# jnbraun/bcnn

Hardware: AMD Instinct MI355X
Metric: images/sec fwd+bwd (higher is better)
Workload: dtype f32; 1 GPU; ResNet-18 224x224 (BASELINE configs[2]), N=128 per GPU, fwd+bwd+SGD through bcnn_net C API; CIFAR-example topology + ImageNet stem, fc-1000; batch_per_gpu=128, global_batch=128, parallelism=dp1, comm=none (one rank)

## Files before the change

bcnn_amd/csrc/batchnorm.hip:

```cpp
#include "chan_reduce.h"
#include "batchnorm.h"
#include "bn_math.h"

namespace bcnn_hip {

#ifdef NT_STORES
#define BN_ST4(p, v) do { typedef float f4_ __attribute__((ext_vector_type(4))); const f4_ t_ = {(v).x, (v).y, (v).z, (v).w}; \
                          __builtin_nontemporal_store(t_, reinterpret_cast<f4_*>(p)); } while (0)
#else
#define BN_ST4(p, v) (*reinterpret_cast<float4*>(p) = (v))
#endif


static float4* bn_consts_scratch(int channels) {
    if (BCNN_EXP_ENV("BCNN_HIP_BN_NO_CONSTS")) return nullptr;
    return scratch_f4(SCRATCH_BN_CONSTS, (size_t)channels * 3);
}
__device__ __forceinline__ void bn_fwd_consts_store(float4* consts, int c, float mean, float var, const float* scale,
                                                    const float* bias) {
    if (!consts) return;
    const BnDiv rs = bn_divisor(sqrtf(var + 0.000001f));
    consts[2 * c] = make_float4(mean, rs.d, rs.r, scale[c]);
    consts[2 * c + 1] = make_float4(bias[c], 0.f, 0.f, 0.f);
}
__device__ __forceinline__ void bn_bwd_consts_store(float4* consts, int c, const float* mean, float var, float sc,
                                                    const float* fwd_bias, float dmean, float dvar, float fM) {
    if (!consts) return;
    const BnDiv rs5 = bn_divisor(sqrtf(var + 0.00001f)), rs6 = bn_divisor(sqrtf(var + 0.000001f));
    consts[3 * c] = make_float4(mean[c], sc, rs5.d, rs5.r);
    consts[3 * c + 1] = make_float4(rs6.d, rs6.r, fwd_bias ? fwd_bias[c] : 0.f, __fdiv_rn(dmean, fM));
    consts[3 * c + 2] = make_float4(dvar, 0.f, 0.f, 0.f);
}

struct StatsF {
    static constexpr int kInFlight = 4;
    const float* x;
    __device__ void operator()(long long off, int, float (&acc)[2]) const {
        const float v = x[off];
        acc[0] += v;
        acc[1] += v * v;
    }
    __device__ void vec4(long long off, int, float (&acc)[2]) const {
        const float4 v = *reinterpret_cast<const float4*>(x + off);
        acc[0] += (v.x + v.y) + (v.z + v.w);
        acc[1] += (v.x * v.x + v.y * v.y) + (v.z * v.z + v.w * v.w);
    }
};

__global__ void bn_stats_finalize_kernel(const float* __restrict__ partials, int C, int splits, int M,
                                         float* __restrict__ saved_mean, float* __restrict__ saved_var,
                                         float* __restrict__ run_mean, float* __restrict__ run_var,
                                         float4* __restrict__ consts, const float* __restrict__ scale,
                                         const float* __restrict__ bias, const float* __restrict__ mean_shift) {
    const int c = blockIdx.x * blockDim.x + threadIdx.x;
    if (c >= C) return;
    double s = 0.0, ss = 0.0;
    for (int i = 0; i < splits; ++i) {
        s += (double)partials[((long long)c * splits + i) * 2 + 0];
        ss += (double)partials[((long long)c * splits + i) * 2 + 1];
    }
    const float inv = 1.0f / (float)M;
    const float mean = __fmul_rn((float)s, inv);
    const float var = __fsub_rn(__fmul_rn((float)ss, inv), __fmul_rn(mean, mean));
    saved_mean[c] = mean;
    saved_var[c] = var;
    const float vis = mean_shift ? __fadd_rn(mean, mean_shift[c]) : mean;
    run_mean[c] = __fadd_rn(__fmul_rn(vis, 0.1f), __fmul_rn(run_mean[c], 0.9f));
    run_var[c] = __fadd_rn(__fmul_rn(var, 0.1f), __fmul_rn(run_var[c], 0.9f));
    bn_fwd_consts_store(consts, c, mean, var, scale, bias);
}

constexpr int kFinalizeThreads = 1024;
__global__ __launch_bounds__(kFinalizeThreads) void bn_stats_finalize_wide_kernel(
    const float* __restrict__ partials, int C, int splits, int M, float* __restrict__ saved_mean,
    float* __restrict__ saved_var, float* __restrict__ run_mean, float* __restrict__ run_var,
    float4* __restrict__ consts, const float* __restrict__ scale, const float* __restrict__ bias,
    const float* __restrict__ mean_shift) {
    constexpr int NW = kFinalizeThreads / 64;
    __shared__ double red[NW][2];
    const int lane = threadIdx.x & 63, wid = threadIdx.x >> 6;
    const int c = blockIdx.x;
    const float2* p = reinterpret_cast<const float2*>(partials) + (long long)c * splits;
    double s = 0.0, ss = 0.0;
    int i = threadIdx.x;
    for (; i + 3 * kFinalizeThreads < splits; i += 4 * kFinalizeThreads) {
        const float2 v0 = p[i], v1 = p[i + kFinalizeThreads], v2 = p[i + 2 * kFinalizeThreads], v3 = p[i + 3 * kFinalizeThreads];
        s += ((double)v0.x + (double)v1.x) + ((double)v2.x + (double)v3.x);
        ss += ((double)v0.y + (double)v1.y) + ((double)v2.y + (double)v3.y);
    }
    for (; i < splits; i += kFinalizeThreads) {
        const float2 v = p[i];
        s += (double)v.x;
        ss += (double)v.y;
    }
#pragma unroll
    for (int o = 32; o > 0; o >>= 1) { s += __shfl_xor(s, o); ss += __shfl_xor(ss, o); }
    if (lane == 0) { red[wid][0] = s; red[wid][1] = ss; }
    __syncthreads();
    if (threadIdx.x != 0) return;
    s = 0.0;
    ss = 0.0;
    for (int w = 0; w < NW; ++w) { s += red[w][0]; ss += red[w][1]; }
    const float inv = 1.0f / (float)M;
    const float mean = __fmul_rn((float)s, inv);
    const float var = __fsub_rn(__fmul_rn((float)ss, inv), __fmul_rn(mean, mean));
    saved_mean[c] = mean;
    saved_var[c] = var;
    const float vis = mean_shift ? __fadd_rn(mean, mean_shift[c]) : mean;
    run_mean[c] = __fadd_rn(__fmul_rn(vis, 0.1f), __fmul_rn(run_mean[c], 0.9f));
    run_var[c] = __fadd_rn(__fmul_rn(var, 0.1f), __fmul_rn(run_var[c], 0.9f));
    bn_fwd_consts_store(consts, c, mean, var, scale, bias);
}

struct BnApplyArgs {
    const float* x;
    float* y;
    float* ws;
    float* xn;
    const float* mean;
    const float* var;
    const float* scale;
    const float* bias;
    int C, HW, predict, act;
    long long total;
    const float* res;
    unsigned res_count;
    int act2;
    const float4* consts;
};

struct BnApplyBody {
    BnApplyArgs a;
    bool al;
    __device__ void operator()(unsigned off, int c, int cnt) const {
        float mean, sc, b;
        BnDiv rs;
        if (a.consts) {
            const float4 k0 = a.consts[2 * c], k1 = a.consts[2 * c + 1];
            mean = k0.x; rs.d = k0.y; rs.r = k0.z; sc = k0.w; b = k1.x;
        } else {
            mean = a.predict ? 0.f : a.mean[c];
            rs = bn_divisor(a.predict ? 1.f : sqrtf(a.var[c] + 0.000001f));
            sc = a.scale[c]; b = a.bias[c];
        }
        const bool side_ws = a.ws && a.ws != a.x, side_xn = a.xn && !a.predict;
        if (cnt == 4 && al && (off & 3u) == 0) {
            const float4 xv = *reinterpret_cast<const float4*>(a.x + off);
            float4 yv, nv;
            yv.x = bn_one(xv.x, mean, rs, sc, b, a.predict, a.act, &nv.x);
            yv.y = bn_one(xv.y, mean, rs, sc, b, a.predict, a.act, &nv.y);
            yv.z = bn_one(xv.z, mean, rs, sc, b, a.predict, a.act, &nv.z);
            yv.w = bn_one(xv.w, mean, rs, sc, b, a.predict, a.act, &nv.w);
            if (side_ws) *reinterpret_cast<float4*>(a.ws + off) = xv;
            if (side_xn) *reinterpret_cast<float4*>(a.xn + off) = nv;
            if (a.res) {
                if (off + 4 <= a.res_count) {
                    const float4 r = *reinterpret_cast<const float4*>(a.res + off);
                    yv.x += r.x; yv.y += r.y; yv.z += r.z; yv.w += r.w;
                } else if (off < a.res_count) {
                    yv.x += a.res[off];
                    if (off + 1 < a.res_count) yv.y += a.res[off + 1];
                    if (off + 2 < a.res_count) yv.z += a.res[off + 2];
                }
                yv.x = act_fwd_cheap(yv.x, a.act2, 0.f); yv.y = act_fwd_cheap(yv.y, a.act2, 0.f);
                yv.z = act_fwd_cheap(yv.z, a.act2, 0.f); yv.w = act_fwd_cheap(yv.w, a.act2, 0.f);
            }
            BN_ST4(a.y + off, yv);
        } else {
            for (int k = 0; k < cnt; ++k) {
                const float xv = a.x[off + k];
                float nv = 0.f;
                float yv = bn_one(xv, mean, rs, sc, b, a.predict, a.act, &nv);
                if (a.res) yv = act_fwd_cheap(yv + (off + k < a.res_count ? a.res[off + k] : 0.f), a.act2, 0.f);
                if (side_ws) a.ws[off + k] = xv;
                if (side_xn) a.xn[off + k] = nv;
                a.y[off + k] = yv;
            }
        }
    }
};

__device__ __forceinline__ float bn_recompute_y(float x, float m, const BnDiv& rs, float sc, float b, int act, const float* res,
                                                unsigned res_count, unsigned long long off) {
    float dummy;
    if (!res) return bn_one(x, m, rs, sc, b, 0, act, &dummy);
    float v = bn_one(x, m, rs, sc, b, 0, BCNN_HIP_ACT_NONE, &dummy);
    if (off < res_count) v += res[off];
    return act_fwd_cheap(v, act, 0.f);
}

struct BwdSumsF {
    static constexpr int kInFlight = 2;
    const float* dy;
    const float* y;
    const float* x;
    const float* mean;
    const float* fwd_bias;
    const float* var;
    const float* scale;
    int act, C, HW;
    const float* res;
    unsigned res_count;
    __device__ float fwd_y(float xv, int c, long long off) const {
        return bn_recompute_y(xv, mean[c], bn_divisor(sqrtf(var[c] + 0.000001f)), scale[c], fwd_bias[c], act, res, res_count,
                              (unsigned long long)off);
    }
    __device__ void operator()(long long off, int c, float (&acc)[2]) const {
        float g = dy[off];
        const float xv = x[off];
        if (act != BCNN_HIP_ACT_NONE) g *= act_bwd_cheap(fwd_bias ? fwd_y(xv, c, off) : y[off], act, 0.f);
        acc[0] += g;
        acc[1] += g * (xv - mean[c]);
    }
    __device__ void vec4(long long off, int c, float (&acc)[2]) const {
        const float m = mean[c];
        float4 g = *reinterpret_cast<const float4*>(dy + off);
        const float4 xv = *reinterpret_cast<const float4*>(x + off);
        if (act != BCNN_HIP_ACT_NONE) {
            float4 yv;
            if (fwd_bias) {
                const BnDiv rs = bn_divisor(sqrtf(var[c] + 0.000001f));
                const float sc = scale[c], b = fwd_bias[c];
                const unsigned long long o = (unsigned long long)off;
                yv.x = bn_recompute_y(xv.x, m, rs, sc, b, act, res, res_count, o);
                yv.y = bn_recompute_y(xv.y, m, rs, sc, b, act, res, res_count, o + 1);
                yv.z = bn_recompute_y(xv.z, m, rs, sc, b, act, res, res_count, o + 2);
                yv.w = bn_recompute_y(xv.w, m, rs, sc, b, act, res, res_count, o + 3);
            } else {
                yv = *reinterpret_cast<const float4*>(y + off);
            }
            g.x *= act_bwd_cheap(yv.x, act, 0.f); g.y *= act_bwd_cheap(yv.y, act, 0.f);
            g.z *= act_bwd_cheap(yv.z, act, 0.f); g.w *= act_bwd_cheap(yv.w, act, 0.f);
        }
        acc[0] += (g.x + g.y) + (g.z + g.w);
        acc[1] += (g.x * (xv.x - m) + g.y * (xv.y - m)) + (g.z * (xv.z - m) + g.w * (xv.w - m));
    }
};

__global__ void bn_bwd_finalize_kernel(const float* __restrict__ partials, int C, int splits,
                                       const float* __restrict__ scale, const float* __restrict__ var,
                                       float* __restrict__ dbias, float* __restrict__ dscales,
                                       float* __restrict__ dmean, float* __restrict__ dvar,
                                       float4* __restrict__ consts, const float* __restrict__ mean,
                                       const float* __restrict__ fwd_bias, float fM) {
    const int c = blockIdx.x * blockDim.x + threadIdx.x;
    if (c >= C) return;
    double s1 = 0.0, s2 = 0.0;
    for (int i = 0; i < splits; ++i) {
        s1 += (double)partials[((long long)c * splits + i) * 2 + 0];
        s2 += (double)partials[((long long)c * splits + i) * 2 + 1];
    }
    const float v = var[c], sc = scale[c];
    dbias[c] += (float)s1;
    dscales[c] += (float)(s2 / (double)sqrtf(v + 0.000001f));
    float md = (float)(s1 * (double)sc);
    float vd = (float)(s2 * (double)sc);
    md *= (-1.0f / sqrtf(v + 0.00001f));
    vd *= -0.5f / (v * sqrtf(v) + 0.00001f);
    dmean[c] = md;
    dvar[c] = vd;
    bn_bwd_consts_store(consts, c, mean, v, sc, fwd_bias, md, vd, fM);
}

__global__ __launch_bounds__(1024) void bn_bwd_finalize_wide_kernel(const float* __restrict__ partials, int C, int splits,
                                                                   const float* __restrict__ scale,
                                                                   const float* __restrict__ var, float* __restrict__ dbias,
                                                                   float* __restrict__ dscales, float* __restrict__ dmean,
                                                                   float* __restrict__ dvar, float4* __restrict__ consts,
                                                                   const float* __restrict__ mean,
                                                                   const float* __restrict__ fwd_bias, float fM) {
    __shared__ double red[16][2];
    const int lane = threadIdx.x & 63, wid = threadIdx.x >> 6, c = blockIdx.x;
    const float2* p = reinterpret_cast<const float2*>(partials) + (long long)c * splits;
    double s1 = 0.0, s2 = 0.0;
    int i = threadIdx.x;
    for (; i + 3 * 1024 < splits; i += 4 * 1024) {
        const float2 v0 = p[i], v1 = p[i + 1024], v2 = p[i + 2048], v3 = p[i + 3072];
        s1 += ((double)v0.x + (double)v1.x) + ((double)v2.x + (double)v3.x);
        s2 += ((double)v0.y + (double)v1.y) + ((double)v2.y + (double)v3.y);
    }
    for (; i < splits; i += 1024) {
        const float2 v = p[i];
        s1 += (double)v.x;
        s2 += (double)v.y;
    }
#pragma unroll
    for (int o = 32; o > 0; o >>= 1) { s1 += __shfl_xor(s1, o); s2 += __shfl_xor(s2, o); }
    if (lane == 0) { red[wid][0] = s1; red[wid][1] = s2; }
    __syncthreads();
    if (threadIdx.x != 0) return;
    s1 = 0.0;
    s2 = 0.0;
    for (int w = 0; w < 16; ++w) { s1 += red[w][0]; s2 += red[w][1]; }
    const float v = var[c], sc = scale[c];
    dbias[c] += (float)s1;
    dscales[c] += (float)(s2 / (double)sqrtf(v + 0.000001f));
    float md = (float)(s1 * (double)sc);
    float vd = (float)(s2 * (double)sc);
    md *= (-1.0f / sqrtf(v + 0.00001f));
    vd *= -0.5f / (v * sqrtf(v) + 0.00001f);
    dmean[c] = md;
    dvar[c] = vd;
    bn_bwd_consts_store(consts, c, mean, v, sc, fwd_bias, md, vd, fM);
}

struct BnBwdApplyArgs {
    float* dy;
    float* dx;
    const float* y;
    const float* x;
    const float* mean;
    const float* var;
    const float* scale;
    const float* dmean;
    const float* dvar;
    const float* fwd_bias;
    int C, HW, act, M;
    long long total;
    int keep_dy;
    const float* res;
    unsigned res_count;
    const float4* consts;
    float rM;
};

struct BnBwdApplyBody {
    BnBwdApplyArgs a;
    bool al;
    __device__ void operator()(unsigned off, int c, int cnt) const {
        const BnDiv fM{(float)a.M, a.rM};
        const bool use_act = a.act != BCNN_HIP_ACT_NONE, use_y = use_act && a.fwd_bias == nullptr;
        float mean, sc, fb, dmm, dv;
        BnDiv rs, rs_fwd;
        if (a.consts) {
            const float4 k0 = a.consts[3 * c], k1 = a.consts[3 * c + 1], k2 = a.consts[3 * c + 2];
            mean = k0.x; sc = k0.y; rs.d = k0.z; rs.r = k0.w;
            rs_fwd.d = k1.x; rs_fwd.r = k1.y; fb = k1.z; dmm = k1.w; dv = k2.x;
        } else {
            mean = a.mean[c]; sc = a.scale[c];
            rs = bn_divisor(sqrtf(a.var[c] + 0.00001f));
            rs_fwd = bn_divisor(use_act && !use_y ? sqrtf(a.var[c] + 0.000001f) : 1.0f);
            fb = a.fwd_bias ? a.fwd_bias[c] : 0.f;
            dmm = __fdiv_rn(a.dmean[c], fM.d); dv = a.dvar[c];
        }
        if (cnt == 4 && al && (off & 3u) == 0) {
            const float4 g = *reinterpret_cast<const float4*>(a.dy + off);
            const float4 xv = *reinterpret_cast<const float4*>(a.x + off);
            float4 yv = make_float4(0.f, 0.f, 0.f, 0.f);
            if (use_y) yv = *reinterpret_cast<const float4*>(a.y + off);
            else if (use_act) {
                yv.x = bn_recompute_y(xv.x, mean, rs_fwd, sc, fb, a.act, a.res, a.res_count, off);
                yv.y = bn_recompute_y(xv.y, mean, rs_fwd, sc, fb, a.act, a.res, a.res_count, off + 1ull);
                yv.z = bn_recompute_y(xv.z, mean, rs_fwd, sc, fb, a.act, a.res, a.res_count, off + 2ull);
                yv.w = bn_recompute_y(xv.w, mean, rs_fwd, sc, fb, a.act, a.res, a.res_count, off + 3ull);
            }
            float4 o;
            o.x = bn_bwd_one(g.x, yv.x, xv.x, mean, rs, sc, dmm, dv, fM, a.act);
            o.y = bn_bwd_one(g.y, yv.y, xv.y, mean, rs, sc, dmm, dv, fM, a.act);
            o.z = bn_bwd_one(g.z, yv.z, xv.z, mean, rs, sc, dmm, dv, fM, a.act);
            o.w = bn_bwd_one(g.w, yv.w, xv.w, mean, rs, sc, dmm, dv, fM, a.act);
            if (!a.keep_dy) BN_ST4(a.dy + off, o);
            if (a.dx) BN_ST4(a.dx + off, o);
        } else {
            for (int k = 0; k < cnt; ++k) {
                const float xk = a.x[off + k];
                const float yk = use_y ? a.y[off + k]
                                       : (use_act ? bn_recompute_y(xk, mean, rs_fwd, sc, fb, a.act, a.res, a.res_count, off + k) : 0.f);
                const float o = bn_bwd_one(a.dy[off + k], yk, xk, mean, rs, sc, dmm, dv, fM, a.act);
                if (!a.keep_dy) a.dy[off + k] = o;
                if (a.dx) a.dx[off + k] = o;
            }
        }
    }
};

void batchnorm_forward_impl(const BnFwdCall& f) {
    const int n = f.e.n, c = f.e.c, hw = f.e.hw, mode = f.mode;
    const long long M = (long long)n * hw, total = M * c;
    if (!total) return;
    const bool have_pre = f.pre && f.pre->splits > 0 && mode == BCNN_HIP_MODE_TRAIN;
    KTimer kt(K_BN_FWD, 0.0, 4.0 * ((have_pre ? 0.0 : 1.0) + (f.stats_only ? 0.0 : 2.0)) * (double)total);
    const int act = act_is_cheap(f.act) ? f.act : BCNN_HIP_ACT_NONE;
    BnApplyArgs a;
    a.x = f.x; a.y = f.y; a.ws = f.workspace; a.xn = f.x_norm; a.scale = f.p.scales; a.bias = f.p.bias;
    a.C = c; a.HW = hw; a.act = act; a.total = total;
    a.res = nullptr; a.res_count = 0; a.act2 = BCNN_HIP_ACT_NONE;
    if (f.res) {
        a.res = f.res->res;
        a.res_count = (unsigned)(f.res->count < (size_t)total ? f.res->count : (size_t)total);
        a.act2 = f.res->act;
    }
    a.predict = (mode == BCNN_HIP_MODE_PREDICT);
    a.mean = f.run.run_mean; a.var = f.run.run_var;
    a.consts = nullptr;
    float4* consts = (mode == BCNN_HIP_MODE_TRAIN && !f.stats_only) ? bn_consts_scratch(c) : nullptr;
    if (mode == BCNN_HIP_MODE_PREDICT) a.ws = nullptr;
    if (mode == BCNN_HIP_MODE_VALID) a.xn = nullptr;
    if (mode == BCNN_HIP_MODE_TRAIN) {
        if (have_pre) {
            bn_stats_finalize_wide_kernel<<<c, kFinalizeThreads, 0, current_stream()>>>(
                f.pre->partials, c, f.pre->splits, (int)M, f.saved_mean, f.saved_var, f.run.run_mean, f.run.run_var, consts,
                f.p.scales, f.p.bias, f.mean_shift);
        } else {
            const int splits = chan_splits(c, M);
            float* part = scratch(SCRATCH_REDUCE, (size_t)c * splits * 2);
            launch_chan_reduce<2>(StatsF{f.x}, c, hw, M, splits, part);
            bn_stats_finalize_kernel<<<ceil_div(c, 256), 256, 0, current_stream()>>>(
                part, c, splits, (int)M, f.saved_mean, f.saved_var, f.run.run_mean, f.run.run_var, consts, f.p.scales, f.p.bias,
                f.mean_shift);
        }
        KERNEL_CHECK();
        a.mean = f.saved_mean; a.var = f.saved_var; a.consts = consts;
    }
    if (f.stats_only) return;
#ifdef BCNN_HIP_EXPERIMENT
    static const int skip_fw = getenv("BCNN_HIP_SKIP_SWEEPS") ? atoi(getenv("BCNN_HIP_SKIP_SWEEPS")) : 0;
    if (!(skip_fw & 4))
#endif
    launch_chan_map(BnApplyBody{a, al16(f.x) && al16(f.y) && al16(a.ws) && al16(a.xn) && al16(a.res)}, n, c, hw);
    if (f.act != act) bcnn_hip_activation_forward(f.y, (size_t)total, f.act, nullptr, hw, c);
}

}

using namespace bcnn_hip;

extern "C" {

void bcnn_hip_batchnorm_forward_stats(const float* x, float* y, float* run_mean, float* run_var, const float* scales,
                                      const float* bias, float* saved_mean, float* saved_var, float* x_norm,
                                      float* workspace, int n, int c, int hw, int mode, int act, const float* stats,
                                      int splits) {
    ConvStats st;
    st.partials = const_cast<float*>(stats); st.splits = stats ? splits : 0; st.capacity = 0;
    BnFwdCall f{};
    f.x = x; f.y = y; f.workspace = workspace; f.x_norm = x_norm; f.mode = mode; f.act = act; f.pre = &st;
    f.e.n = n; f.e.c = c; f.e.hw = hw; f.p.scales = scales; f.p.bias = bias;
    f.saved_mean = saved_mean; f.saved_var = saved_var; f.run.run_mean = run_mean; f.run.run_var = run_var;
    batchnorm_forward_impl(f);
}

void bcnn_hip_batchnorm_forward(const float* x, float* y, float* run_mean, float* run_var,
                                const float* scales, const float* bias, float* saved_mean,
                                float* saved_var, float* x_norm, float* workspace, int n, int c, int hw,
                                int mode, int act) {
    bcnn_hip_batchnorm_forward_stats(x, y, run_mean, run_var, scales, bias, saved_mean, saved_var, x_norm, workspace, n, c, hw,
                                     mode, act, nullptr, 0);
}

void bcnn_hip_batchnorm_forward_stats_only(const float* x, float* run_mean, float* run_var, const float* scales,
                                           const float* bias, float* saved_mean, float* saved_var, int n, int c, int hw,
                                           const float* stats, int splits) {
    ConvStats st;
    st.partials = const_cast<float*>(stats); st.splits = stats ? splits : 0; st.capacity = 0;
    BnFwdCall f{};
    f.x = x; f.mode = BCNN_HIP_MODE_TRAIN; f.act = BCNN_HIP_ACT_NONE; f.pre = &st; f.stats_only = true;
    f.e.n = n; f.e.c = c; f.e.hw = hw; f.p.scales = scales; f.p.bias = bias;
    f.saved_mean = saved_mean; f.saved_var = saved_var; f.run.run_mean = run_mean; f.run.run_var = run_var;
    batchnorm_forward_impl(f);
}

}

namespace bcnn_hip {
void batchnorm_backward_sums(const BnBwdCall& b) {
    const int c = b.e.c, hw = b.e.hw;
    const long long M = (long long)b.e.n * hw;
    const int splits = chan_splits(c, M);
    float* part = scratch(SCRATCH_REDUCE, (size_t)c * splits * 2);
    BwdSumsF f;
    f.dy = b.dout ? b.dout : b.dy; f.y = b.y; f.x = b.workspace; f.mean = b.s.mean; f.act = b.act; f.C = c; f.HW = hw;
    f.fwd_bias = b.p.bias; f.var = b.s.var; f.scale = b.p.scales; f.res = b.res; f.res_count = (unsigned)b.res_count;
#ifdef BCNN_HIP_EXPERIMENT
    static const int skip_exp = getenv("BCNN_HIP_SKIP_C1_SUMS") ? 1 : 0;
    static const int skip_all = getenv("BCNN_HIP_SKIP_SWEEPS") ? atoi(getenv("BCNN_HIP_SKIP_SWEEPS")) : 0;
    if (!(skip_all & 1))
    if (!(skip_exp && b.res == nullptr && b.act == BCNN_HIP_ACT_RELU && ((hw == 3136 && c == 64) || (hw == 784 && c == 128))))
#endif
    launch_chan_reduce<2>(f, c, hw, M, splits, part);
    bn_bwd_finalize_kernel<<<ceil_div(c, 256), 256, 0, current_stream()>>>(part, c, splits, b.p.scales, b.s.var, b.g.dbias,
                                                                          b.g.dscales, b.g.dmean, b.g.dvar, b.consts, b.s.mean,
                                                                          b.p.bias, b.consts_fM > 0.f ? b.consts_fM : (float)M);
    KERNEL_CHECK();
}

static void batchnorm_backward_apply(const BnBwdCall& b) {
    const long long M = (long long)b.e.n * b.e.hw, total = M * b.e.c;
    BnBwdApplyArgs a;
    a.consts = b.consts;
    a.rM = 1.0f / (float)M;
    a.dy = b.dout ? const_cast<float*>(b.dout) : b.dy;
    a.dx = (b.dx && b.dx != a.dy) ? b.dx : nullptr; a.y = b.y; a.x = b.workspace;
    a.mean = b.s.mean; a.var = b.s.var; a.scale = b.p.scales; a.dmean = b.g.dmean; a.dvar = b.g.dvar;
    a.C = b.e.c; a.HW = b.e.hw; a.act = b.act; a.M = (int)M; a.total = total; a.fwd_bias = b.p.bias;
    a.keep_dy = b.dout != nullptr; a.res = b.res; a.res_count = (unsigned)b.res_count;
#ifdef BCNN_HIP_EXPERIMENT
    static const int skip_bw = getenv("BCNN_HIP_SKIP_SWEEPS") ? atoi(getenv("BCNN_HIP_SKIP_SWEEPS")) : 0;
    if (skip_bw & 2) return;
#endif
    launch_chan_map(BnBwdApplyBody{a, al16(a.dy) && al16(a.dx) && al16(b.workspace) && al16(b.y)}, b.e.n, b.e.c, b.e.hw);
}

__global__ __launch_bounds__(256) void bn_residual_grad_kernel(const float* __restrict__ out, const float* __restrict__ dout,
                                                               float* __restrict__ dres, unsigned count, int act) {
    for (unsigned i = blockIdx.x * 256u + threadIdx.x; i < count; i += gridDim.x * 256u)
        dres[i] += dout[i] * act_bwd_cheap(out[i], act, 0.f);
}

void batchnorm_backward_impl(const BnBwdCall& call) {
    BnBwdCall b = call;
    const int c = b.e.c, hw = b.e.hw;
    const long long M = (long long)b.e.n * hw, total = M * c;
    if (!total) return;
    if (!b.dout && (b.act == BCNN_HIP_ACT_NONE || !act_bwd_is_cheap(b.act))) b.p.bias = nullptr;
    const bool reads_y = b.act != BCNN_HIP_ACT_NONE && !b.p.bias;
    KTimer kt(K_BN_BWD, 0.0, 4.0 * (b.dout ? 5.0 : b.sums ? (reads_y ? 4.0 : 3.0) : (reads_y ? 7.0 : 5.0)) * (double)total);
    if (b.dout) {
        b.res_count = b.res_count < (size_t)total ? b.res_count : (size_t)total;
        if (b.dres && b.res_count) {
            bn_residual_grad_kernel<<<stream_grid(b.res_count, 256), 256, 0, current_stream()>>>(b.y, b.dout, b.dres,
                                                                                                 (unsigned)b.res_count, b.act);
            KERNEL_CHECK();
        }
    } else if (!act_bwd_is_cheap(b.act)) {
        bcnn_hip_activation_backward(b.y, b.dy, (size_t)total, b.act, nullptr, nullptr, hw, c);
        b.act = BCNN_HIP_ACT_NONE;
    }
    b.consts = bn_consts_scratch(c);
    if (b.sums) {
        bn_bwd_finalize_wide_kernel<<<c, 1024, 0, current_stream()>>>(b.sums, c, b.splits, b.p.scales, b.s.var, b.g.dbias, b.g.dscales,
                                                                      b.g.dmean, b.g.dvar, b.consts, b.s.mean, b.p.bias, (float)M);
        KERNEL_CHECK();
    } else {
        batchnorm_backward_sums(b);
    }
    batchnorm_backward_apply(b);
}

}

extern "C" {

void bcnn_hip_batchnorm_apply(const float* x, float* y, const float* scales, const float* bias, const float* saved_mean,
                              const float* saved_var, int n, int c, int hw, int act) {
    const long long total = (long long)n * hw * c;
    if (!total) return;
    BnApplyArgs a;
    a.x = x; a.y = y; a.ws = nullptr; a.xn = nullptr; a.scale = scales; a.bias = bias; a.mean = saved_mean; a.var = saved_var;
    a.C = c; a.HW = hw; a.act = act_is_cheap(act) ? act : BCNN_HIP_ACT_NONE; a.total = total; a.predict = 0;
    a.res = nullptr; a.res_count = 0; a.act2 = BCNN_HIP_ACT_NONE; a.consts = nullptr;
    launch_chan_map(BnApplyBody{a, al16(x) && al16(y)}, n, c, hw);
    if (a.act != act) bcnn_hip_activation_forward(y, (size_t)total, act, nullptr, hw, c);
}

void bcnn_hip_batchnorm_backward_finalize(const float* sums, int splits, const float* scales, float* dscales, float* dbias,
                                          const float* saved_var, float* dmean, float* dvar, int c) {
    if (c <= 0 || splits <= 0) return;
    bn_bwd_finalize_wide_kernel<<<c, 1024, 0, current_stream()>>>(sums, c, splits, scales, saved_var, dbias, dscales, dmean,
                                                                  dvar, nullptr, nullptr, nullptr, 1.0f);
    KERNEL_CHECK();
}

void bcnn_hip_batchnorm_backward_sums(const float* dy, const float* scales, float* dscales, float* dbias,
                                      const float* saved_mean, const float* saved_var, float* dmean, float* dvar,
                                      const float* x, int n, int c, int hw) {
    const long long total = (long long)n * hw * c;
    if (!total) return;
    KTimer kt(K_BN_BWD, 0.0, 4.0 * 2.0 * (double)total);
    BnBwdCall b{};
    b.dout = dy; b.workspace = x; b.act = BCNN_HIP_ACT_NONE; b.e.n = n; b.e.c = c; b.e.hw = hw;
    b.p.scales = scales; b.s.mean = saved_mean; b.s.var = saved_var;
    b.g.dscales = dscales; b.g.dbias = dbias; b.g.dmean = dmean; b.g.dvar = dvar;
    batchnorm_backward_sums(b);
}

void bcnn_hip_batchnorm_backward_apply(float* dy, float* dx, const float* scales, const float* saved_mean,
                                       const float* saved_var, const float* dmean, const float* dvar, const float* x,
                                       int n, int c, int hw) {
    if (!(long long)n * hw * c) return;
    BnBwdCall b{};
    b.dy = dy; b.dx = dx; b.workspace = x; b.act = BCNN_HIP_ACT_NONE; b.e.n = n; b.e.c = c; b.e.hw = hw;
    b.p.scales = scales; b.s.mean = saved_mean; b.s.var = saved_var;
    b.g.dmean = const_cast<float*>(dmean); b.g.dvar = const_cast<float*>(dvar);
    batchnorm_backward_apply(b);
}

void bcnn_hip_batchnorm_backward(float* dy, float* dx, const float* y, int act, const float* scales,
                                 float* dscales, float* dbias, const float* saved_mean,
                                 const float* saved_var, float* dmean, float* dvar, const float* x_norm,
                                 const float* workspace, int n, int c, int hw) {
    (void)x_norm;
    BnBwdCall b{};
    b.dy = dy; b.dx = dx; b.y = y; b.workspace = workspace; b.act = act; b.e.n = n; b.e.c = c; b.e.hw = hw;
    b.p.scales = scales; b.s.mean = saved_mean; b.s.var = saved_var;
    b.g.dscales = dscales; b.g.dbias = dbias; b.g.dmean = dmean; b.g.dvar = dvar;
    batchnorm_backward_impl(b);
}

}
```

Baseline: 14140 images/s.

## Fuse BN stats finalize with per-channel apply in one channel-block kernel

Adds per-channel kernels where one 1024-thread block per channel loads its slice into registers, finalizes the statistics (forward) or gradient sums (backward) in shared memory, then applies normalization. This removes a separate finalize launch and overlaps the initial loads with the reduction. It is enabled for forward when M is at most 32768 and C is at least the CU count. Backward defaults to disabled since its max is 0. Risk: only C blocks are launched, which may leave the GPU underused for small C, and the data walk is serial per channel.

```diff
diff --git a/bcnn_amd/csrc/batchnorm.hip b/bcnn_amd/csrc/batchnorm.hip
--- a/bcnn_amd/csrc/batchnorm.hip
+++ b/bcnn_amd/csrc/batchnorm.hip
@@ -16,20 +16,32 @@
     if (BCNN_EXP_ENV("BCNN_HIP_BN_NO_CONSTS")) return nullptr;
     return scratch_f4(SCRATCH_BN_CONSTS, (size_t)channels * 3);
 }
+struct BnFwdConsts { float4 k0, k1; };
+struct BnBwdConsts { float4 k0, k1, k2; };
+__device__ __forceinline__ BnFwdConsts bn_fwd_consts_make(float mean, float var, float sc, float b) {
+    const BnDiv rs = bn_divisor(sqrtf(var + 0.000001f));
+    return BnFwdConsts{make_float4(mean, rs.d, rs.r, sc), make_float4(b, 0.f, 0.f, 0.f)};
+}
+__device__ __forceinline__ BnBwdConsts bn_bwd_consts_make(float mean, float var, float sc, float fb, float dmean, float dvar,
+                                                          float fM) {
+    const BnDiv rs5 = bn_divisor(sqrtf(var + 0.00001f)), rs6 = bn_divisor(sqrtf(var + 0.000001f));
+    return BnBwdConsts{make_float4(mean, sc, rs5.d, rs5.r), make_float4(rs6.d, rs6.r, fb, __fdiv_rn(dmean, fM)),
+                       make_float4(dvar, 0.f, 0.f, 0.f)};
+}
 __device__ __forceinline__ void bn_fwd_consts_store(float4* consts, int c, float mean, float var, const float* scale,
                                                     const float* bias) {
     if (!consts) return;
-    const BnDiv rs = bn_divisor(sqrtf(var + 0.000001f));
-    consts[2 * c] = make_float4(mean, rs.d, rs.r, scale[c]);
-    consts[2 * c + 1] = make_float4(bias[c], 0.f, 0.f, 0.f);
+    const BnFwdConsts k = bn_fwd_consts_make(mean, var, scale[c], bias[c]);
+    consts[2 * c] = k.k0;
+    consts[2 * c + 1] = k.k1;
 }
 __device__ __forceinline__ void bn_bwd_consts_store(float4* consts, int c, const float* mean, float var, float sc,
                                                     const float* fwd_bias, float dmean, float dvar, float fM) {
     if (!consts) return;
-    const BnDiv rs5 = bn_divisor(sqrtf(var + 0.00001f)), rs6 = bn_divisor(sqrtf(var + 0.000001f));
-    consts[3 * c] = make_float4(mean[c], sc, rs5.d, rs5.r);
-    consts[3 * c + 1] = make_float4(rs6.d, rs6.r, fwd_bias ? fwd_bias[c] : 0.f, __fdiv_rn(dmean, fM));
-    consts[3 * c + 2] = make_float4(dvar, 0.f, 0.f, 0.f);
+    const BnBwdConsts k = bn_bwd_consts_make(mean[c], var, sc, fwd_bias ? fwd_bias[c] : 0.f, dmean, dvar, fM);
+    consts[3 * c] = k.k0;
+    consts[3 * c + 1] = k.k1;
+    consts[3 * c + 2] = k.k2;
 }
 
 struct StatsF {
@@ -71,15 +83,14 @@
 }
 
 constexpr int kFinalizeThreads = 1024;
-__global__ __launch_bounds__(kFinalizeThreads) void bn_stats_finalize_wide_kernel(
-    const float* __restrict__ partials, int C, int splits, int M, float* __restrict__ saved_mean,
-    float* __restrict__ saved_var, float* __restrict__ run_mean, float* __restrict__ run_var,
-    float4* __restrict__ consts, const float* __restrict__ scale, const float* __restrict__ bias,
-    const float* __restrict__ mean_shift) {
+__device__ __forceinline__ void bn_stats_finalize_wide(const float* __restrict__ partials, int c, int splits, int M,
+                                                       float* __restrict__ saved_mean, float* __restrict__ saved_var,
+                                                       float* __restrict__ run_mean, float* __restrict__ run_var,
+                                                       float4* __restrict__ consts, const float* __restrict__ scale,
+                                                       const float* __restrict__ bias, const float* __restrict__ mean_shift,
+                                                       double (*red)[2], float4* lds) {
     constexpr int NW = kFinalizeThreads / 64;
-    __shared__ double red[NW][2];
     const int lane = threadIdx.x & 63, wid = threadIdx.x >> 6;
-    const int c = blockIdx.x;
     const float2* p = reinterpret_cast<const float2*>(partials) + (long long)c * splits;
     double s = 0.0, ss = 0.0;
     int i = threadIdx.x;
@@ -110,6 +121,20 @@
     run_mean[c] = __fadd_rn(__fmul_rn(vis, 0.1f), __fmul_rn(run_mean[c], 0.9f));
     run_var[c] = __fadd_rn(__fmul_rn(var, 0.1f), __fmul_rn(run_var[c], 0.9f));
     bn_fwd_consts_store(consts, c, mean, var, scale, bias);
+    if (lds) {
+        const BnFwdConsts k = bn_fwd_consts_make(mean, var, scale[c], bias[c]);
+        lds[0] = k.k0;
+        lds[1] = k.k1;
+    }
+}
+__global__ __launch_bounds__(kFinalizeThreads) void bn_stats_finalize_wide_kernel(
+    const float* __restrict__ partials, int C, int splits, int M, float* __restrict__ saved_mean,
+    float* __restrict__ saved_var, float* __restrict__ run_mean, float* __restrict__ run_var,
+    float4* __restrict__ consts, const float* __restrict__ scale, const float* __restrict__ bias,
+    const float* __restrict__ mean_shift) {
+    __shared__ double red[kFinalizeThreads / 64][2];
+    bn_stats_finalize_wide(partials, blockIdx.x, splits, M, saved_mean, saved_var, run_mean, run_var, consts, scale, bias,
+                           mean_shift, red, nullptr);
 }
 
 struct BnApplyArgs {
@@ -237,19 +262,12 @@
     }
 };
 
-__global__ void bn_bwd_finalize_kernel(const float* __restrict__ partials, int C, int splits,
-                                       const float* __restrict__ scale, const float* __restrict__ var,
-                                       float* __restrict__ dbias, float* __restrict__ dscales,
-                                       float* __restrict__ dmean, float* __restrict__ dvar,
-                                       float4* __restrict__ consts, const float* __restrict__ mean,
-                                       const float* __restrict__ fwd_bias, float fM) {
-    const int c = blockIdx.x * blockDim.x + threadIdx.x;
-    if (c >= C) return;
-    double s1 = 0.0, s2 = 0.0;
-    for (int i = 0; i < splits; ++i) {
-        s1 += (double)partials[((long long)c * splits + i) * 2 + 0];
-        s2 += (double)partials[((long long)c * splits + i) * 2 + 1];
-    }
+__device__ __forceinline__ void bn_bwd_finalize_one(double s1, double s2, int c, const float* __restrict__ scale,
+                                                    const float* __restrict__ var, float* __restrict__ dbias,
+                                                    float* __restrict__ dscales, float* __restrict__ dmean,
+                                                    float* __restrict__ dvar, float4* __restrict__ consts,
+                                                    const float* __restrict__ mean, const float* __restrict__ fwd_bias, float fM,
+                                                    float4* lds) {
     const float v = var[c], sc = scale[c];
     dbias[c] += (float)s1;
     dscales[c] += (float)(s2 / (double)sqrtf(v + 0.000001f));
@@ -260,8 +278,60 @@
     dmean[c] = md;
     dvar[c] = vd;
     bn_bwd_consts_store(consts, c, mean, v, sc, fwd_bias, md, vd, fM);
-}
-
+    if (lds) {
+        const BnBwdConsts k = bn_bwd_consts_make(mean[c], v, sc, fwd_bias ? fwd_bias[c] : 0.f, md, vd, fM);
+        lds[0] = k.k0;
+        lds[1] = k.k1;
+        lds[2] = k.k2;
+    }
+}
+__device__ __forceinline__ void bn_bwd_sum_partials(const float* __restrict__ partials, int c, int splits, double& s1, double& s2) {
+    s1 = 0.0;
+    s2 = 0.0;
+    for (int i = 0; i < splits; ++i) {
+        s1 += (double)partials[((long long)c * splits + i) * 2 + 0];
+        s2 += (double)partials[((long long)c * splits + i) * 2 + 1];
+    }
+}
+__global__ void bn_bwd_finalize_kernel(const float* __restrict__ partials, int C, int splits,
+                                       const float* __restrict__ scale, const float* __restrict__ var,
+                                       float* __restrict__ dbias, float* __restrict__ dscales,
+                                       float* __restrict__ dmean, float* __restrict__ dvar,
+                                       float4* __restrict__ consts, const float* __restrict__ mean,
+                                       const float* __restrict__ fwd_bias, float fM) {
+    const int c = blockIdx.x * blockDim.x + threadIdx.x;
+    if (c >= C) return;
+    double s1, s2;
+    bn_bwd_sum_partials(partials, c, splits, s1, s2);
+    bn_bwd_finalize_one(s1, s2, c, scale, var, dbias, dscales, dmean, dvar, consts, mean, fwd_bias, fM, nullptr);
+}
+
+__device__ __forceinline__ void bn_bwd_reduce_wide(const float* __restrict__ partials, int c, int splits, double (*red)[2],
+                                                   double& s1, double& s2) {
+    const int lane = threadIdx.x & 63, wid = threadIdx.x >> 6;
+    const float2* p = reinterpret_cast<const float2*>(partials) + (long long)c * splits;
+    s1 = 0.0;
+    s2 = 0.0;
+    int i = threadIdx.x;
+    for (; i + 3 * 1024 < splits; i += 4 * 1024) {
+        const float2 v0 = p[i], v1 = p[i + 1024], v2 = p[i + 2048], v3 = p[i + 3072];
+        s1 += ((double)v0.x + (double)v1.x) + ((double)v2.x + (double)v3.x);
+        s2 += ((double)v0.y + (double)v1.y) + ((double)v2.y + (double)v3.y);
+    }
+    for (; i < splits; i += 1024) {
+        const float2 v = p[i];
+        s1 += (double)v.x;
+        s2 += (double)v.y;
+    }
+#pragma unroll
+    for (int o = 32; o > 0; o >>= 1) { s1 += __shfl_xor(s1, o); s2 += __shfl_xor(s2, o); }
+    if (lane == 0) { red[wid][0] = s1; red[wid][1] = s2; }
+    __syncthreads();
+    if (threadIdx.x != 0) return;
+    s1 = 0.0;
+    s2 = 0.0;
+    for (int w = 0; w < 16; ++w) { s1 += red[w][0]; s2 += red[w][1]; }
+}
 __global__ __launch_bounds__(1024) void bn_bwd_finalize_wide_kernel(const float* __restrict__ partials, int C, int splits,
                                                                    const float* __restrict__ scale,
                                                                    const float* __restrict__ var, float* __restrict__ dbias,
@@ -270,38 +340,10 @@
                                                                    const float* __restrict__ mean,
                                                                    const float* __restrict__ fwd_bias, float fM) {
     __shared__ double red[16][2];
-    const int lane = threadIdx.x & 63, wid = threadIdx.x >> 6, c = blockIdx.x;
-    const float2* p = reinterpret_cast<const float2*>(partials) + (long long)c * splits;
-    double s1 = 0.0, s2 = 0.0;
-    int i = threadIdx.x;
-    for (; i + 3 * 1024 < splits; i += 4 * 1024) {
-        const float2 v0 = p[i], v1 = p[i + 1024], v2 = p[i + 2048], v3 = p[i + 3072];
-        s1 += ((double)v0.x + (double)v1.x) + ((double)v2.x + (double)v3.x);
-        s2 += ((double)v0.y + (double)v1.y) + ((double)v2.y + (double)v3.y);
-    }
-    for (; i < splits; i += 1024) {
-        const float2 v = p[i];
-        s1 += (double)v.x;
-        s2 += (double)v.y;
-    }
-#pragma unroll
-    for (int o = 32; o > 0; o >>= 1) { s1 += __shfl_xor(s1, o); s2 += __shfl_xor(s2, o); }
-    if (lane == 0) { red[wid][0] = s1; red[wid][1] = s2; }
-    __syncthreads();
+    double s1, s2;
+    bn_bwd_reduce_wide(partials, blockIdx.x, splits, red, s1, s2);
     if (threadIdx.x != 0) return;
-    s1 = 0.0;
-    s2 = 0.0;
-    for (int w = 0; w < 16; ++w) { s1 += red[w][0]; s2 += red[w][1]; }
-    const float v = var[c], sc = scale[c];
-    dbias[c] += (float)s1;
-    dscales[c] += (float)(s2 / (double)sqrtf(v + 0.000001f));
-    float md = (float)(s1 * (double)sc);
-    float vd = (float)(s2 * (double)sc);
-    md *= (-1.0f / sqrtf(v + 0.00001f));
-    vd *= -0.5f / (v * sqrtf(v) + 0.00001f);
-    dmean[c] = md;
-    dvar[c] = vd;
-    bn_bwd_consts_store(consts, c, mean, v, sc, fwd_bias, md, vd, fM);
+    bn_bwd_finalize_one(s1, s2, blockIdx.x, scale, var, dbias, dscales, dmean, dvar, consts, mean, fwd_bias, fM, nullptr);
 }
 
 struct BnBwdApplyArgs {
@@ -374,6 +416,256 @@
     }
 };
 
+constexpr int kChanThreads = kFinalizeThreads;
+
+template <int V>
+__device__ __forceinline__ void chan_ld(const float* p, float (&v)[V]) {
+    if constexpr (V == 4) {
+        const float4 t = *reinterpret_cast<const float4*>(p);
+        v[0] = t.x; v[1] = t.y; v[2] = t.z; v[3] = t.w;
+    } else {
+        v[0] = *p;
+    }
+}
+template <int V>
+__device__ __forceinline__ void chan_st(float* p, const float (&v)[V]) {
+    if constexpr (V == 4) {
+        const float4 t = make_float4(v[0], v[1], v[2], v[3]);
+        BN_ST4(p, t);
+    } else {
+        *p = v[0];
+    }
+}
+
+template <int V, int U, class Op>
+struct ChanBatch {
+    unsigned R, T, sp, si, img, base;
+    unsigned u, n, i;
+    unsigned off[U];
+    bool ok[U];
+    typename Op::template Regs<V> r[U];
+    __device__ __forceinline__ ChanBatch(int N, int C, int HW, int c) {
+        R = (unsigned)HW / V; T = (unsigned)N * R;
+        sp = kChanThreads / R; si = kChanThreads - sp * R;
+        img = (unsigned)C * (unsigned)HW; base = (unsigned)c * (unsigned)HW;
+        u = threadIdx.x; n = u / R; i = u - n * R;
+    }
+    __device__ __forceinline__ void load(const Op& op) {
+#pragma unroll
+        for (int k = 0; k < U; ++k) {
+            ok[k] = u < T;
+            off[k] = ok[k] ? base + n * img + i * V : base;
+            op.template load<V>(off[k], r[k]);
+            u += kChanThreads; n += sp; i += si;
+            if (i >= R) { i -= R; ++n; }
+        }
+    }
+    __device__ __forceinline__ void apply(const Op& op) {
+#pragma unroll
+        for (int k = 0; k < U; ++k)
+            if (ok[k]) op.template apply<V>(off[k], r[k]);
+    }
+};
+
+template <int V, int U, class Op, class Phase1>
+__device__ __forceinline__ void channel_walk(Op& op, const Phase1& phase1, int N, int C, int HW, int c) {
+    ChanBatch<V, U, Op> b(N, C, HW, c);
+    b.load(op);
+    phase1(op);
+    b.apply(op);
+    while (b.u < b.T) {
+        b.load(op);
+        b.apply(op);
+    }
+}
+
+template <bool RES>
+struct BnFwdChanOp {
+    BnApplyArgs a;
+    const float* dummy;
+    float mean, sc, b;
+    BnDiv rs;
+    template <int V> struct Regs { float x[V]; float r[RES ? V : 1]; };
+    __device__ __forceinline__ void set(const float4* k) {
+        mean = k[0].x; rs.d = k[0].y; rs.r = k[0].z; sc = k[0].w; b = k[1].x;
+    }
+    template <int V>
+    __device__ __forceinline__ void load(unsigned off, Regs<V>& g) const {
+        chan_ld<V>(a.x + off, g.x);
+        if constexpr (RES) chan_ld<V>(off + V <= a.res_count ? a.res + off : dummy, g.r);
+    }
+    template <int V>
+    __device__ __forceinline__ void apply(unsigned off, const Regs<V>& g) const {
+        float y[V], nv[V];
+#pragma unroll
+        for (int j = 0; j < V; ++j) y[j] = bn_one(g.x[j], mean, rs, sc, b, 0, a.act, &nv[j]);
+        if (a.ws && a.ws != a.x) chan_st<V>(a.ws + off, g.x);
+        if (a.xn) chan_st<V>(a.xn + off, nv);
+        if constexpr (RES) {
+            float r[V];
+#pragma unroll
+            for (int j = 0; j < V; ++j) r[j] = g.r[j];
+            if (V > 1 && off < a.res_count && off + V > a.res_count) {
+#pragma unroll
+                for (int j = 0; j < V; ++j)
+                    if (off + j < a.res_count) r[j] = a.res[off + j];
+            }
+#pragma unroll
+            for (int j = 0; j < V; ++j) {
+                if (off + j < a.res_count) y[j] += r[j];
+                y[j] = act_fwd_cheap(y[j], a.act2, 0.f);
+            }
+        }
+        chan_st<V>(a.y + off, y);
+    }
+};
+
+struct BnFwdChanStats {
+    const float* partials;
+    int splits, M;
+    float *saved_mean, *saved_var, *run_mean, *run_var;
+    float4* consts;
+    const float* mean_shift;
+};
+
+template <bool RES>
+__global__ __launch_bounds__(kChanThreads) void bn_fwd_channel_kernel(const BnApplyArgs a, const BnFwdChanStats st, int N,
+                                                                      bool vec) {
+    __shared__ double red[kFinalizeThreads / 64][2];
+    __shared__ float4 kc[2];
+    const int c = blockIdx.x;
+    BnFwdChanOp<RES> op;
+    op.a = a;
+    op.dummy = a.x + (unsigned)c * (unsigned)a.HW;
+    const auto phase1 = [&](BnFwdChanOp<RES>& o) {
+        bn_stats_finalize_wide(st.partials, c, st.splits, st.M, st.saved_mean, st.saved_var, st.run_mean, st.run_var, st.consts,
+                               a.scale, a.bias, st.mean_shift, red, kc);
+        __syncthreads();
+        o.set(kc);
+    };
+    if (vec) channel_walk<4, 4>(op, phase1, N, a.C, a.HW, c);
+    else channel_walk<1, 8>(op, phase1, N, a.C, a.HW, c);
+}
+
+template <int MODE>
+struct BnBwdChanOp {
+    BnBwdApplyArgs a;
+    float* dres;
+    const float* dummy;
+    float mean, sc, fb, dmm, dv;
+    BnDiv rs, rs_fwd, fM;
+    template <int V> struct Regs { float g[V], x[V]; float y[MODE == 1 ? V : 1]; float r[MODE == 2 ? V : 1]; float d[MODE == 2 ? V : 1]; };
+    __device__ __forceinline__ void set(const float4* k) {
+        mean = k[0].x; sc = k[0].y; rs.d = k[0].z; rs.r = k[0].w;
+        rs_fwd.d = k[1].x; rs_fwd.r = k[1].y; fb = k[1].z; dmm = k[1].w; dv = k[2].x;
+        fM.d = (float)a.M; fM.r = a.rM;
+    }
+    template <int V>
+    __device__ __forceinline__ void load(unsigned off, Regs<V>& g) const {
+        chan_ld<V>(a.dy + off, g.g);
+        chan_ld<V>(a.x + off, g.x);
+        if constexpr (MODE == 1) chan_ld<V>(a.y + off, g.y);
+        if constexpr (MODE == 2) {
+            const bool in = off + V <= a.res_count;
+            chan_ld<V>(in ? a.res + off : dummy, g.r);
+            chan_ld<V>(in && dres ? dres + off : dummy, g.d);
+        }
+    }
+    template <int V>
+    __device__ __forceinline__ void apply(unsigned off, const Regs<V>& g) const {
+        const bool use_act = a.act != BCNN_HIP_ACT_NONE;
+        float yv[V], o[V];
+        if constexpr (MODE == 2) {
+            float r[V], d[V];
+#pragma unroll
+            for (int j = 0; j < V; ++j) { r[j] = g.r[j]; d[j] = g.d[j]; }
+            const bool ends = V > 1 && off < a.res_count && off + V > a.res_count;
+            if (ends) {
+#pragma unroll
+                for (int j = 0; j < V; ++j)
+                    if (off + j < a.res_count) { r[j] = a.res[off + j]; if (dres) d[j] = dres[off + j]; }
+            }
+#pragma unroll
+            for (int j = 0; j < V; ++j) {
+                yv[j] = 0.f;
+                if (use_act) {
+                    float dummy_xn;
+                    float v = bn_one(g.x[j], mean, rs_fwd, sc, fb, 0, BCNN_HIP_ACT_NONE, &dummy_xn);
+                    if (off + j < a.res_count) v += r[j];
+                    yv[j] = act_fwd_cheap(v, a.act, 0.f);
+                }
+                d[j] += g.g[j] * act_bwd_cheap(yv[j], a.act, 0.f);
+            }
+            if (dres) {
+                if (off + V <= a.res_count) {
+                    chan_st<V>(dres + off, d);
+                } else if (ends) {
+#pragma unroll
+                    for (int j = 0; j < V; ++j)
+                        if (off + j < a.res_count) dres[off + j] = d[j];
+                }
+            }
+        } else {
+#pragma unroll
+            for (int j = 0; j < V; ++j)
+                yv[j] = MODE == 1 ? g.y[j] : (use_act ? bn_recompute_y(g.x[j], mean, rs_fwd, sc, fb, a.act, nullptr, 0, 0) : 0.f);
+        }
+#pragma unroll
+        for (int j = 0; j < V; ++j) o[j] = bn_bwd_one(g.g[j], yv[j], g.x[j], mean, rs, sc, dmm, dv, fM, a.act);
+        if (!a.keep_dy) chan_st<V>(a.dy + off, o);
+        if (a.dx) chan_st<V>(a.dx + off, o);
+    }
+};
+
+struct BnBwdChanSums {
+    const float* partials;
+    int splits;
+    float *dbias, *dscales, *dmean, *dvar;
+    float4* consts;
+    float fM;
+};
+
+template <bool WIDE, int MODE>
+__global__ __launch_bounds__(kChanThreads) void bn_bwd_channel_kernel(const BnBwdApplyArgs a, const BnBwdChanSums sm,
+                                                                      float* dres, int N, bool vec) {
+    __shared__ double red[16][2];
+    __shared__ float4 kc[3];
+    const int c = blockIdx.x;
+    BnBwdChanOp<MODE> op;
+    op.a = a;
+    op.dres = dres;
+    op.dummy = a.x + (unsigned)c * (unsigned)a.HW;
+    const auto phase1 = [&](BnBwdChanOp<MODE>& o) {
+        double s1 = 0.0, s2 = 0.0;
+        if constexpr (WIDE) bn_bwd_reduce_wide(sm.partials, c, sm.splits, red, s1, s2);
+        if (threadIdx.x == 0) {
+            if constexpr (!WIDE) bn_bwd_sum_partials(sm.partials, c, sm.splits, s1, s2);
+            bn_bwd_finalize_one(s1, s2, c, a.scale, a.var, sm.dbias, sm.dscales, sm.dmean, sm.dvar, sm.consts, a.mean, a.fwd_bias,
+                                sm.fM, kc);
+        }
+        __syncthreads();
+        o.set(kc);
+    };
+    if (vec) channel_walk<4, 4>(op, phase1, N, a.C, a.HW, c);
+    else channel_walk<1, 8>(op, phase1, N, a.C, a.HW, c);
+}
+
+#ifndef BN_CHANNEL_FWD_MAX
+#define BN_CHANNEL_FWD_MAX 32768
+#endif
+#ifndef BN_CHANNEL_BWD_MAX
+#define BN_CHANNEL_BWD_MAX 0
+#endif
+static bool bn_channel_rule(int n, int c, int hw, bool backward) {
+    const long long M = (long long)n * hw;
+    if (M * c > 0xffff0000LL) return false;
+    if (const char* e = BCNN_EXP_ENV("BCNN_HIP_BN_CHANNEL")) {
+        if (e[0] == '0') return false;
+        if (e[0] == '2') return true;
+    }
+    return c >= kCUs && M <= (backward ? BN_CHANNEL_BWD_MAX : BN_CHANNEL_FWD_MAX);
+}
+
 void batchnorm_forward_impl(const BnFwdCall& f) {
     const int n = f.e.n, c = f.e.c, hw = f.e.hw, mode = f.mode;
     const long long M = (long long)n * hw, total = M * c;
@@ -396,6 +688,16 @@
     float4* consts = (mode == BCNN_HIP_MODE_TRAIN && !f.stats_only) ? bn_consts_scratch(c) : nullptr;
     if (mode == BCNN_HIP_MODE_PREDICT) a.ws = nullptr;
     if (mode == BCNN_HIP_MODE_VALID) a.xn = nullptr;
+    if (have_pre && !f.stats_only && f.act == act && bn_channel_rule(n, c, hw, false)) {
+        trace_kernel("bn_fwd_channel_kernel");
+        const BnFwdChanStats st{f.pre->partials, f.pre->splits, (int)M, f.saved_mean, f.saved_var, f.run.run_mean,
+                                f.run.run_var, consts, f.mean_shift};
+        const bool vec = (hw & 3) == 0 && al16(f.x) && al16(f.y) && al16(a.ws) && al16(a.xn) && al16(a.res);
+        if (a.res) bn_fwd_channel_kernel<true><<<c, kChanThreads, 0, current_stream()>>>(a, st, n, vec);
+        else bn_fwd_channel_kernel<false><<<c, kChanThreads, 0, current_stream()>>>(a, st, n, vec);
+        KERNEL_CHECK();
+        return;
+    }
     if (mode == BCNN_HIP_MODE_TRAIN) {
         if (have_pre) {
             bn_stats_finalize_wide_kernel<<<c, kFinalizeThreads, 0, current_stream()>>>(
@@ -413,6 +715,7 @@
         a.mean = f.saved_mean; a.var = f.saved_var; a.consts = consts;
     }
     if (f.stats_only) return;
+    trace_kernel("bn_fwd_sweep");
 #ifdef BCNN_HIP_EXPERIMENT
     static const int skip_fw = getenv("BCNN_HIP_SKIP_SWEEPS") ? atoi(getenv("BCNN_HIP_SKIP_SWEEPS")) : 0;
     if (!(skip_fw & 4))
@@ -463,7 +766,7 @@
 }
 
 namespace bcnn_hip {
-void batchnorm_backward_sums(const BnBwdCall& b) {
+static float* bn_bwd_sums_sweep(const BnBwdCall& b, int* splits_out) {
     const int c = b.e.c, hw = b.e.hw;
     const long long M = (long long)b.e.n * hw;
     const int splits = chan_splits(c, M);
@@ -471,6 +774,7 @@
     BwdSumsF f;
     f.dy = b.dout ? b.dout : b.dy; f.y = b.y; f.x = b.workspace; f.mean = b.s.mean; f.act = b.act; f.C = c; f.HW = hw;
     f.fwd_bias = b.p.bias; f.var = b.s.var; f.scale = b.p.scales; f.res = b.res; f.res_count = (unsigned)b.res_count;
+    *splits_out = splits;
 #ifdef BCNN_HIP_EXPERIMENT
     static const int skip_exp = getenv("BCNN_HIP_SKIP_C1_SUMS") ? 1 : 0;
     static const int skip_all = getenv("BCNN_HIP_SKIP_SWEEPS") ? atoi(getenv("BCNN_HIP_SKIP_SWEEPS")) : 0;
@@ -478,13 +782,21 @@
     if (!(skip_exp && b.res == nullptr && b.act == BCNN_HIP_ACT_RELU && ((hw == 3136 && c == 64) || (hw == 784 && c == 128))))
 #endif
     launch_chan_reduce<2>(f, c, hw, M, splits, part);
+    return part;
+}
+
+void batchnorm_backward_sums(const BnBwdCall& b) {
+    const int c = b.e.c;
+    const long long M = (long long)b.e.n * b.e.hw;
+    int splits = 0;
+    const float* part = bn_bwd_sums_sweep(b, &splits);
     bn_bwd_finalize_kernel<<<ceil_div(c, 256), 256, 0, current_stream()>>>(part, c, splits, b.p.scales, b.s.var, b.g.dbias,
                                                                           b.g.dscales, b.g.dmean, b.g.dvar, b.consts, b.s.mean,
                                                                           b.p.bias, b.consts_fM > 0.f ? b.consts_fM : (float)M);
     KERNEL_CHECK();
 }
 
-static void batchnorm_backward_apply(const BnBwdCall& b) {
+static BnBwdApplyArgs bn_bwd_apply_args(const BnBwdCall& b) {
     const long long M = (long long)b.e.n * b.e.hw, total = M * b.e.c;
     BnBwdApplyArgs a;
     a.consts = b.consts;
@@ -494,11 +806,32 @@
     a.mean = b.s.mean; a.var = b.s.var; a.scale = b.p.scales; a.dmean = b.g.dmean; a.dvar = b.g.dvar;
     a.C = b.e.c; a.HW = b.e.hw; a.act = b.act; a.M = (int)M; a.total = total; a.fwd_bias = b.p.bias;
     a.keep_dy = b.dout != nullptr; a.res = b.res; a.res_count = (unsigned)b.res_count;
+    return a;
+}
+
+static void batchnorm_backward_apply(const BnBwdCall& b) {
+    const BnBwdApplyArgs a = bn_bwd_apply_args(b);
 #ifdef BCNN_HIP_EXPERIMENT
     static const int skip_bw = getenv("BCNN_HIP_SKIP_SWEEPS") ? atoi(getenv("BCNN_HIP_SKIP_SWEEPS")) : 0;
     if (skip_bw & 2) return;
 #endif
     launch_chan_map(BnBwdApplyBody{a, al16(a.dy) && al16(a.dx) && al16(b.workspace) && al16(b.y)}, b.e.n, b.e.c, b.e.hw);
+}
+
+static void batchnorm_backward_channel(const BnBwdCall& b, const float* partials, int splits, bool wide) {
+    const BnBwdApplyArgs a = bn_bwd_apply_args(b);
+    const int n = b.e.n, c = b.e.c;
+    const BnBwdChanSums sm{partials, splits, b.g.dbias, b.g.dscales, b.g.dmean, b.g.dvar, b.consts, (float)a.M};
+    float* dres = (b.dout && b.res_count) ? b.dres : nullptr;
+    const bool vec = (a.HW & 3) == 0 && al16(a.dy) && al16(a.dx) && al16(a.x) && al16(a.y) && al16(a.res) && al16(dres);
+    const int mode = a.res ? 2 : (a.act != BCNN_HIP_ACT_NONE && !a.fwd_bias) ? 1 : 0;
+    trace_kernel("bn_bwd_channel_kernel");
+    hipStream_t s = current_stream();
+#define BN_BWD_CHAN(W, MD) bn_bwd_channel_kernel<W, MD><<<c, kChanThreads, 0, s>>>(a, sm, dres, n, vec)
+    if (wide) { if (mode == 2) BN_BWD_CHAN(true, 2); else if (mode == 1) BN_BWD_CHAN(true, 1); else BN_BWD_CHAN(true, 0); }
+    else      { if (mode == 2) BN_BWD_CHAN(false, 2); else if (mode == 1) BN_BWD_CHAN(false, 1); else BN_BWD_CHAN(false, 0); }
+#undef BN_BWD_CHAN
+    KERNEL_CHECK();
 }
 
 __global__ __launch_bounds__(256) void bn_residual_grad_kernel(const float* __restrict__ out, const float* __restrict__ dout,
@@ -515,9 +848,10 @@
     if (!b.dout && (b.act == BCNN_HIP_ACT_NONE || !act_bwd_is_cheap(b.act))) b.p.bias = nullptr;
     const bool reads_y = b.act != BCNN_HIP_ACT_NONE && !b.p.bias;
     KTimer kt(K_BN_BWD, 0.0, 4.0 * (b.dout ? 5.0 : b.sums ? (reads_y ? 4.0 : 3.0) : (reads_y ? 7.0 : 5.0)) * (double)total);
+    const bool chan = bn_channel_rule(b.e.n, c, hw, true) && (b.dout ? (b.res && b.p.bias) : act_bwd_is_cheap(b.act));
     if (b.dout) {
         b.res_count = b.res_count < (size_t)total ? b.res_count : (size_t)total;
-        if (b.dres && b.res_count) {
+        if (b.dres && b.res_count && !chan) {
             bn_residual_grad_kernel<<<stream_grid(b.res_count, 256), 256, 0, current_stream()>>>(b.y, b.dout, b.dres,
                                                                                                  (unsigned)b.res_count, b.act);
             KERNEL_CHECK();
@@ -527,6 +861,13 @@
         b.act = BCNN_HIP_ACT_NONE;
     }
     b.consts = bn_consts_scratch(c);
+    if (chan) {
+        int splits = b.splits;
+        const float* part = b.sums ? b.sums : bn_bwd_sums_sweep(b, &splits);
+        batchnorm_backward_channel(b, part, splits, b.sums != nullptr);
+        return;
+    }
+    trace_kernel("bn_bwd_sweep");
     if (b.sums) {
         bn_bwd_finalize_wide_kernel<<<c, 1024, 0, current_stream()>>>(b.sums, c, b.splits, b.p.scales, b.s.var, b.g.dbias, b.g.dscales,
                                                                       b.g.dmean, b.g.dvar, b.consts, b.s.mean, b.p.bias, (float)M);
```

Result: no change. 14160 images/s, median of 6 (+0.2%).
